# ElesionKyrie/Extreme-Video-Compression-With-Prediction-Using-Pre-trainded-Diffusion-Models-

Measured on AMD Instinct MI355X. Metric: decoded frames/sec (128x128x30) at q3, higher is better.
Workload: dtype f32

## Files before the change

### extreme-video-compression-with-prediction-using-pre-trainded-diffusion-models-_amd/build.py

```python
import os
import shutil
import subprocess
import sys
from concurrent.futures import ThreadPoolExecutor

HERE = os.path.dirname(os.path.abspath(__file__))
CSRC = os.path.join(HERE, "csrc")
LIBDIR = os.path.join(HERE, "lib")
OBJDIR = os.path.join(HERE, "build")
INCLUDE = os.path.join(os.path.dirname(HERE), "include")
HIP_SOURCES = ["conv_igemm.hip", "nin_gemm.hip", "attention.hip", "norm.hip", "fir.hip", "elementwise.hip", "gdn.hip", "stride2.hip", "lpips.hip", "i3d.hip", "frames.hip", "noise.hip", "yuv.hip", "rate.hip", "ssim.hip", "metric.hip", "inception.hip", "resample.hip", "tile.hip", "api.hip"]
ARCH = "gfx950"


def _newer(target, deps):
    if not os.path.exists(target):
        return True
    t = os.path.getmtime(target)
    return any(os.path.getmtime(d) > t for d in deps)


def _run(cmd):
    r = subprocess.run(cmd, capture_output=True, text=True)
    if r.returncode != 0:
        raise RuntimeError("build failed: %s\n%s\n%s" % (" ".join(cmd), r.stdout, r.stderr))


def hipcc_path():
    for c in (os.environ.get("HIPCC"), shutil.which("hipcc"), "/opt/rocm/bin/hipcc"):
        if c and os.path.exists(c):
            return c
    raise RuntimeError("hipcc not found (ROCm toolchain required to build libevc_hip.so)")


# ... 34 lines not shown
```

### extreme-video-compression-with-prediction-using-pre-trainded-diffusion-models-_amd/lib.py

```python
import ctypes
import math
import os
from ctypes import POINTER, c_char_p, c_double, c_float, c_int, c_int32, c_longlong, c_uint, c_uint8, c_ulonglong, c_void_p

import numpy as np
import torch

HERE = os.path.dirname(os.path.abspath(__file__))
HIP_SO = os.path.join(HERE, "lib", "libevc_hip.so")
if os.environ.get("EVC_HIP_SO"):
    HIP_SO = os.path.abspath(os.environ["EVC_HIP_SO"])
RANS_SO = os.path.join(HERE, "lib", "libevc_rans.so")

ACT_NONE, ACT_SILU, ACT_RELU = 0, 1, 2
ARITH_F32, ARITH_BF16X6, ARITH_F16X3 = 0, 1, 2
_ARITH_NAMES = {"f32": ARITH_F32, "bf16x6": ARITH_BF16X6, "f16x3": ARITH_F16X3}
_ARITH_DTYPES = {ARITH_F32: torch.float32, ARITH_BF16X6: torch.bfloat16, ARITH_F16X3: torch.float16}


def _arith_policy():
    name = os.environ.get("EVC_CONV_ARITH", "f16x3").lower()
    if name not in _ARITH_NAMES:
        raise ValueError(f"EVC_CONV_ARITH must be one of {sorted(_ARITH_NAMES)}, got {name!r}")
    return _ARITH_NAMES[name]
# ... 24 lines not shown
                ("out_scale", c_float), ("act_out", c_int),
                ("out", c_void_p), ("ld_out", c_int),
                ("B", c_int), ("H", c_int), ("W", c_int), ("Co", c_int), ("KH", c_int), ("KW", c_int),
                ("splits", c_int), ("stats_out", c_void_p), ("arith", c_int), ("in_bound", c_void_p),
                ("x2_src0", c_void_p), ("x2_src1", c_void_p), ("x2_C0", c_int), ("x2_C1", c_int), ("x2_ld0", c_int),
                ("x2_ld1", c_int), ("x2_w_packed", c_void_p), ("x2_bound", c_void_p), ("invariant", c_int)]


class ConvPlan(ctypes.Structure):
    _fields_ = [("kernel", ctypes.c_char * 96), ("tile_m", c_int), ("tile_n", c_int), ("splits", c_int),
                ("steps_per_split", c_int), ("cut_chunk", c_int), ("tail_tiles", c_int), ("tail_splits", c_int),
                ("stats_runs", c_int), ("fused_1x1", c_int)]


class NinArgs(ctypes.Structure):
    _fields_ = [("x", c_void_p), ("x1", c_void_p), ("Ci", c_int), ("Co", c_int), ("coef_a", c_void_p), ("coef_s", c_void_p),
                ("in_bound", c_void_p), ("w_packed", c_void_p), ("arith", c_int), ("bias", c_void_p), ("res", c_void_p),
                ("out_scale", c_float), ("act_out", c_int), ("out", c_void_p), ("stats_out", c_void_p),
                ("B", c_int), ("H", c_int), ("W", c_int), ("tile", c_int)]


class NinPlan(ctypes.Structure):
    _fields_ = [("kernel", ctypes.c_char * 64), ("tile_m", c_int), ("tile_n", c_int), ("stages", c_int), ("stats_runs", c_int)]


class AttentionPlan(ctypes.Structure):
    _fields_ = [("kernel", ctypes.c_char * 64), ("waves", c_int), ("kparts", c_int), ("tiles_per_part", c_int),
                ("kv_planes", c_int), ("merge", c_int), ("short_seq", c_int),
                ("lds_bytes", c_longlong), ("parts_bytes", c_longlong), ("ws_bytes", c_longlong)]


HIP_SYMBOLS = {
    "evc_version": (c_char_p, []),
    "evc_arch": (c_char_p, []),
    "evc_device_ok": (c_int, []),
    "evc_clock_probe": (c_int, [c_void_p, c_int, c_void_p, c_void_p]),
    "evc_im2col_nchw_f32": (c_int, [c_void_p, c_void_p] + [c_int] * 9 + [c_void_p, c_void_p, c_void_p]),
    "evc_maxpool3s2_nhwc_f32": (c_int, [c_void_p, c_void_p, c_int, c_int, c_int, c_int, c_void_p]),
    "evc_lpips_layer_f32": (c_int, [c_void_p, c_void_p, c_void_p, c_void_p, c_int, c_int, c_int, c_int, c_void_p]),
    "evc_maxpool2d_nhwc_f32": (c_int, [c_void_p, c_void_p] + [c_int] * 7 + [c_void_p]),
    "evc_lpips_map_f32": (c_int, [c_void_p, c_void_p, c_void_p, c_void_p, c_int, c_int, c_int, c_void_p]),
    "evc_lpips_map_mean_f32": (c_int, [c_void_p, c_void_p, c_int, c_int, c_int, c_void_p]),
    "evc_lpips_upsample_add_f32": (c_int, [c_void_p, c_void_p] + [c_int] * 6 + [c_void_p]),
    "evc_i3d_stem_im2col_f32": (c_int, [c_void_p, c_void_p] + [c_int] * 17 + [c_void_p]),
    "evc_maxpool3d_same_nthwc_f32": (c_int, [c_void_p, c_void_p] + [c_int] * 11 + [c_void_p]),
    "evc_i3d_head_f32": (c_int, [c_void_p] * 4 + [c_int] * 6 + [c_void_p]),
# ... 42 lines not shown
    "evc_gdn_workspace_bytes": (c_longlong, [c_int, c_int, c_int, c_int]),
    "evc_gdn_f32": (c_int, [c_void_p, c_void_p, c_int, c_void_p, c_void_p, c_void_p, c_int, c_int, c_int, c_int, c_int,
                            c_int, c_void_p]),
    "evc_affine_act_nhwc_f32": (c_int, [c_void_p, c_void_p, c_void_p, c_void_p, c_int, c_int, c_int, c_int, c_int,
                                        c_int, c_void_p]),
    "evc_conv_co_pad": (c_int, [c_int]),
    "evc_conv_packed_floats": (c_longlong, [c_int, c_int, c_int, c_int]),
    "evc_conv_pack_weights_f32": (c_int, [c_void_p, c_void_p, c_int, c_int, c_int, c_int, c_void_p]),
    "evc_conv_packed_bytes": (c_longlong, [c_int, c_int, c_int, c_int, c_int]),
    "evc_conv_pack_weights": (c_int, [c_void_p, c_void_p, c_int, c_int, c_int, c_int, c_int, c_void_p]),
    "evc_conv_set_option": (c_int, [c_char_p, c_int]),
    "evc_spade_act_nhwc_f32": (c_int, [c_void_p, c_void_p, c_void_p, c_void_p, c_int, c_void_p, c_void_p, c_int, c_void_p,
                                       c_void_p, c_int, c_void_p, c_int, c_int, c_int, c_int, c_int, c_void_p]),
    "evc_conv_choose_splits": (c_int, [POINTER(ConvArgs)]),
    "evc_conv_kernel_name": (c_int, [POINTER(ConvArgs), c_char_p, c_int]),
    "evc_conv_fused_1x1_supported": (c_int, [POINTER(ConvArgs)]),
    "evc_conv_stats_splits": (c_int, [POINTER(ConvArgs)]),
    "evc_conv_workspace_bytes": (c_longlong, [POINTER(ConvArgs)]),
    "evc_conv2d_nhwc_f32": (c_int, [POINTER(ConvArgs), c_void_p, c_void_p]),
    "evc_conv2d_nhwc_profiled_f32": (c_int, [POINTER(ConvArgs), c_void_p, c_void_p, c_void_p, c_void_p]),
    "evc_nin_gemm_supported": (c_int, [POINTER(NinArgs)]),
    "evc_nin_gemm_plan_query": (c_int, [POINTER(NinArgs), POINTER(NinPlan)]),
    "evc_nin_gemm_f32": (c_int, [POINTER(NinArgs), c_void_p]),
    "evc_attention_f32": (c_int, [c_void_p, c_void_p, c_void_p, c_int, c_void_p, c_int, c_int, c_int, c_int, c_int,
                                  c_float, c_void_p]),
    "evc_attention_workspace_bytes": (c_longlong, [c_int, c_int, c_int, c_int]),
    "evc_attention_set_option": (c_int, [c_char_p, c_int]),
    "evc_attention_plan_query": (c_int, [c_int, c_int, c_int, c_int, c_int, c_int, c_int, POINTER(AttentionPlan)]),
    "evc_attention_ws_f32": (c_int, [c_void_p, c_void_p, c_void_p, c_int, c_void_p, c_int, c_int, c_int, c_int, c_int,
                                     c_float, c_void_p, c_void_p]),
    "evc_frame_group_norm_f32": (c_int, [c_void_p] * 4 + [c_int] * 5 + [c_float, c_void_p]),
    "evc_frame_attention_f32": (c_int, [c_void_p, c_int, c_void_p, c_int] + [c_int] * 5 + [c_float, c_void_p]),
    "evc_frame_mix_f32": (c_int, [c_void_p] * 4 + [c_int] * 3 + [c_longlong, c_void_p]),
    "evc_frame_taps_f32": (c_int, [c_void_p, c_void_p] + [c_int] * 4 + [c_void_p]),
    "evc_ddpm_step_f32": (c_int, [c_void_p, c_void_p, c_void_p, c_longlong] + [c_float] * 5 + [c_int, c_void_p]),
    "evc_ddim_step_f32": (c_int, [c_void_p, c_void_p, c_longlong] + [c_float] * 4 + [c_int, c_void_p]),
    "evc_axpy_f32": (c_int, [c_void_p, c_void_p, c_void_p, c_longlong, c_float, c_void_p]),
    "evc_pndm_transfer_f32": (c_int, [c_void_p, c_void_p, c_void_p, c_longlong, c_float, c_float, c_float, c_int,
                                      c_void_p]),
    "evc_lincomb4_f32": (c_int, [c_void_p] * 5 + [c_longlong] + [c_float] * 4 + [c_void_p]),
    "evc_scale_clamp_f32": (c_int, [c_void_p, c_void_p, c_longlong, c_float, c_float, c_int, c_float, c_float,
                                    c_void_p]),
    "evc_gate_residual_f32": (c_int, [c_void_p, c_void_p, c_void_p, c_void_p, c_longlong, c_void_p]),
    "evc_elic_gather_params_f32": (c_int, [c_void_p] + [c_int] * 8 + [c_void_p, c_int, c_void_p, c_void_p,
                                                                       c_void_p]),
    "evc_elic_scatter_symbols_f32": (c_int, [c_void_p, c_void_p, c_void_p] + [c_int] * 7 + [c_void_p]),
# ... 717 lines not shown
    L = hip_lib()
    B, H, W, Ci = x.shape
    assert x.is_contiguous() and x.dtype == torch.float32 and (res is None or (res.is_contiguous() and res.shape == (B, H, W, Co)))
    if out is None:
        out = torch.empty((B, H, W, Co), device=x.device, dtype=torch.float32)
    assert out.is_contiguous() and out.shape == (B, H, W, Co)
    ca, cs = coef if coef is not None else (None, None)
    assert ca is None or (ca.shape == (B, Ci) and cs.shape == (B, Ci) and ca.is_contiguous() and cs.is_contiguous())
    a = NinArgs(x=ptr(x), x1=None, Ci=Ci, Co=Co, coef_a=ptr(ca), coef_s=ptr(cs), in_bound=_word(in_bound),
                w_packed=ptr(w_packed), arith=packed_arith(w_packed), bias=ptr(bias), res=ptr(res), out_scale=float(out_scale),
                act_out=ACT_NONE, out=ptr(out), B=B, H=H, W=W, tile=tile)
    plan = NinPlan()
    _check(L.evc_nin_gemm_plan_query(ctypes.byref(a), ctypes.byref(plan)), "evc_nin_gemm_plan_query")
    stats = None
    if want_stats:
        stats = torch.empty((B, plan.stats_runs, Co, 2), device=x.device, dtype=torch.float32)
        a.stats_out = ptr(stats)
    _check(L.evc_nin_gemm_f32(ctypes.byref(a), stream_ptr()), "evc_nin_gemm_f32")
    if NIN_PROFILE is not None:
        NIN_PROFILE.append(dict(kernel=plan.kernel.decode(), tile=(plan.tile_m, plan.tile_n), shape=(B, H, W, Ci, Co),
                                coef=coef is not None, bound=in_bound is not None, res=res is not None, stats=bool(want_stats)))
    return (out, stats) if want_stats else out


def attention_set_option(name, value):
    if hip_lib(require_device=False).evc_attention_set_option(name.encode(), int(value)) != 0:
        raise EvcKernelError(f"unknown attention option {name!r}")


ATTN_PROFILE = None


def attention_plan(B, heads, N, D, with_bounds=False, have_ws=None, invariant=False):
    L = hip_lib(require_device=False)
    if have_ws is None:
        nbytes = (L.evc_attention_invariant_workspace_bytes if invariant else L.evc_attention_workspace_bytes)(B, heads, N, D)
        have_ws = nbytes > 0
    out = AttentionPlan()
    _check(L.evc_attention_plan_query(B, heads, N, D, int(bool(with_bounds)), int(bool(have_ws)), int(bool(invariant)),
                                      ctypes.byref(out)), "evc_attention_plan_query")
    return dict(kernel=out.kernel.decode(), waves=out.waves, kparts=out.kparts, tiles_per_part=out.tiles_per_part,
                kv_planes=bool(out.kv_planes), merge=bool(out.merge), short_seq=bool(out.short_seq),
                lds_bytes=out.lds_bytes, parts_bytes=out.parts_bytes, ws_bytes=out.ws_bytes)


def attention(qkv, C, heads, out=None, bounds=None, invariant=False, ws=None):
# ... 537 lines not shown
```

### extreme-video-compression-with-prediction-using-pre-trainded-diffusion-models-_amd/scorenet.py

```python
import math
from types import SimpleNamespace

import numpy as np
import torch

from . import lib as L

FIR_K = np.outer([1, 3, 3, 1], [1, 3, 3, 1]).astype(np.float32)
FIR_K /= FIR_K.sum()
INV_SQRT2 = float(np.float32(1.0) / np.sqrt(np.float32(2.0)))


def num_groups(ch):
    g = min(ch // 4, 32)
    while ch % g != 0:
        g -= 1
    return g


def dims_from_config(config):
    m, d = config.model, config.data
    return SimpleNamespace(ngf=m.ngf, ch_mult=list(m.ch_mult), num_res_blocks=m.num_res_blocks,
                           attn_resolutions=list(m.attn_resolutions), n_head_channels=m.n_head_channels,
                           image_size=d.image_size, channels=d.channels, num_frames=d.num_frames,
# ... 180 lines not shown
        self._unfused = set()
        self._site_of = {}
        self._set_site_args()
        self.demote_seconds = 0.0
        self._rows = {}
        self._row_tensors = {}
        self._table = torch.zeros((256, self.ss_total), device=self.device, dtype=torch.float32)
        self._n_rows = 0
        self.use_graphs = use_graphs
        self._graphs = {}
        self._f16_raw = L.bounded_arith() == L.ARITH_F16X3
        import os
        self.overlap_skip = os.environ.get("EVC_OVERLAP_SKIP", "1") != "0"
        self.fuse_skip = self._f16_raw and os.environ.get("EVC_FUSE_SKIP", "1") != "0"
        self._side_streams = {}
        self._bounds_by_stream = {}
        self._bounds = None
        self._bound_next = 0
        self._bound_batch = 1
        if demote:
            self.demote(demote)

    def _conv(self, *a, **kw):
        return L.conv2d_nhwc(*a, invariant=self.batch_invariant, **kw)

    def _act(self, t, stats=None):
        return _Act(t, stats, invariant=self.batch_invariant)

    def _gn(self, *a, **kw):
        return L.gn_coeffs(*a, invariant=self.batch_invariant, **kw)

    def _mbound(self, *a, **kw):
        return L.moments_bound(*a, invariant=self.batch_invariant, **kw)

    def _attention(self, *a, **kw):
        return L.attention(*a, invariant=self.batch_invariant, **kw)

    def _fuse_ok(self, *a, **kw):
        return L.conv_fused_1x1_supported(*a, invariant=self.batch_invariant, **kw)

    def invariant_view(self):
        import copy
        if self.batch_invariant:
            return self
        if self.SPADE or self.ARCH != "unetmore" or self.noise_in_cond:
            raise NotImplementedError("batch_invariant is built for the concat-conditioned score network (ScoreNet) only")
        if self._demoted:
# ... 286 lines not shown
        if qkvb is None:
            obound = None
            qkv = self._proj(x.t, e["wqkv"], 3 * C, e["bqkv"], coef=coef)
        else:
            qkv, qst = self._proj(x.t, e["wqkv"], 3 * C, e["bqkv"], coef=coef, want_stats=True)
            self._mbound(qst, 0, C, qkvb, site=self._site("attn_qkv", i))
            obound = _f16_only(e["wo"], qkvb.view(B, 3)[:, 2].contiguous() if self.batch_invariant else qkvb[2:3])
        o = self._attention(qkv.view(B, H * W, 3 * C), C, heads, bounds=None if i in self._attn_f32 else qkvb)
        return self._act(*self._proj(o.view(B, H, W, C), e["wo"], C, e["bo"], res=x.t, out_scale=INV_SQRT2, want_stats=True,
                                     in_bound=obound))

    nin_gemm = True

    def _proj(self, x, w, Co, bias, coef=None, res=None, out_scale=1.0, want_stats=False, in_bound=None):
        B, H, W, Ci = x.shape
        plain = not self.batch_invariant and not self.SPADE and self.ARCH == "unetmore"
        if self.nin_gemm and plain and L.packed_arith(w) == L.ARITH_F16X3 and \
                L.nin_gemm_supported(B, H, W, Ci, Co, coef=coef is not None, bound=in_bound is not None):
            return L.nin_gemm(x, w, Co, bias=bias, coef=coef, res=res, out_scale=out_scale, in_bound=in_bound,
                              want_stats=want_stats)
        return self._conv(x, w, Co, 1, 1, bias=bias, coef=coef, res=res, out_scale=out_scale, want_stats=want_stats,
                          in_bound=in_bound)

    @torch.no_grad()
    def forward_rows(self, x, rows, cond=None):
        if self.batch_invariant and self._demoted:
            raise ValueError("batch-invariant mode does not combine with demoted sites (range recovery)")
        return self._forward_rows(x, rows, cond)

    def _forward_rows(self, x, rows, cond=None):
        d = self.d
        prog = self.program
        B, _, H, W = x.shape
        self._bound_batch = B if self.batch_invariant else 1
        nb = 256 * self._bound_batch
        if self._f16_raw:
            if torch.cuda.is_current_stream_capturing():
                self._bounds = torch.empty(nb, device=self.device, dtype=torch.int32)
            else:
                key = torch.cuda.current_stream().cuda_stream
                self._bounds = self._bounds_by_stream.get(key)
                if self._bounds is None or self._bounds.numel() != nb:
                    self._bounds = self._bounds_by_stream[key] = torch.empty(nb, device=self.device, dtype=torch.int32)
            self._bounds.zero_()
            self._bound_next = 0
        taps = getattr(self, "taps", None)
# ... 119 lines not shown
```

### include/evc_hip.h

```cpp
#ifndef EVC_HIP_H
#define EVC_HIP_H

#ifdef __cplusplus
extern "C" {
#endif

#define EVC_OK 0
#define EVC_EINVAL (-1)
#define EVC_EUNSUPPORTED (-2)
#define EVC_ELAUNCH (-3)

#define EVC_ACT_NONE 0
#define EVC_ACT_SILU 1
#define EVC_ACT_RELU 2

#define EVC_ARITH_F32 0
#define EVC_ARITH_BF16X6 1
#define EVC_ARITH_F16X3 2

const char* evc_version(void);
const char* evc_arch(void);
int evc_device_ok(void);

int evc_clock_probe(unsigned long long* out2, int spin_us, const unsigned* stop, void* stream);
// ... 93 lines not shown

int evc_conv2d_nhwc_profiled_f32(const evc_conv_args* a, float* ws, void* stream, void* ev_start, void* ev_conv_end);

typedef struct {
    const float* x; const float* x1;
    int Ci; int Co;
    const float* coef_a; const float* coef_s;
    const unsigned* in_bound;
    const float* w_packed; int arith;
    const float* bias; const float* res;
    float out_scale; int act_out;
    float* out; float* stats_out;
    int B; int H; int W;
    int tile;
} evc_nin_args;
typedef struct {
    char kernel[64];
    int tile_m, tile_n, stages, stats_runs;
} evc_nin_plan;
int evc_nin_gemm_supported(const evc_nin_args* a);
int evc_nin_gemm_plan_query(const evc_nin_args* a, evc_nin_plan* out);
int evc_nin_gemm_f32(const evc_nin_args* a, void* stream);

int evc_attention_f32(const float* q, const float* k, const float* v, int ld_qkv, float* out, int ld_out, int B,
                      int heads, int N, int D, float scale, void* stream);
long long evc_attention_workspace_bytes(int B, int heads, int N, int D);
int evc_attention_set_option(const char* name, int value);
int evc_attention_ws_f32(const float* q, const float* k, const float* v, int ld_qkv, float* out, int ld_out, int B,
                         int heads, int N, int D, float scale, float* ws, void* stream);

int evc_attention_f16x3_f32(const float* q, const float* k, const float* v, int ld_qkv, float* out, int ld_out, int B,
                            int heads, int N, int D, float scale, const unsigned* bounds, float* ws, void* stream);

typedef struct {
    char kernel[64];
    int waves, kparts, tiles_per_part, kv_planes, merge, short_seq;
    long long lds_bytes, parts_bytes, ws_bytes;
} evc_attention_plan;
int evc_attention_plan_query(int B, int heads, int N, int D, int with_bounds, int have_ws, int invariant,
                             evc_attention_plan* out);

int evc_frame_group_norm_f32(const float* x, float* y, const float* gamma, const float* beta, int B, int N, int HW, int C,
                             int groups, float eps, void* stream);
int evc_frame_attention_f32(const float* qkv, int ld_qkv, float* out, int ld_out, int B, int N, int HW, int C, int heads,
                            float scale, void* stream);
int evc_frame_mix_f32(const float* x, float* y, const float* w, const float* bias, int B, int N, int M, long long inner,
// ... 112 lines not shown
```

Before: 37.86.

## Add specialized small-spatial 3x3 conv kernel with split-K across waves

Adds a dedicated HIP kernel for 3x3 convolutions on small spatial maps that tiles 64 output pixels per workgroup, splits the channel dimension across four waves with an LDS cross-wave reduction, double-buffers activations in LDS and prefetches weights per tap. It also fuses the affine+SiLU input transform, an optional extra 1x1 (x2) input path, residual and stats into the kernel. ScoreNet now routes eligible f16x3 3x3 convs to this kernel instead of the generic implicit-GEMM path. The aim is to cut under-occupancy and launch inefficiency of the generic kernel on small, low-workgroup-count layers. The risk is extra reduction and synchronisation overhead and heuristics that pick poorly for some shapes.

Result: no change. 38.24, median of 6 (+1.0%).

```diff
diff --git a/extreme-video-compression-with-prediction-using-pre-trainded-diffusion-models-_amd/build.py b/extreme-video-compression-with-prediction-using-pre-trainded-diffusion-models-_amd/build.py
--- a/extreme-video-compression-with-prediction-using-pre-trainded-diffusion-models-_amd/build.py
+++ b/extreme-video-compression-with-prediction-using-pre-trainded-diffusion-models-_amd/build.py
@@ -9,7 +9,7 @@
 LIBDIR = os.path.join(HERE, "lib")
 OBJDIR = os.path.join(HERE, "build")
 INCLUDE = os.path.join(os.path.dirname(HERE), "include")
-HIP_SOURCES = ["conv_igemm.hip", "nin_gemm.hip", "attention.hip", "norm.hip", "fir.hip", "elementwise.hip", "gdn.hip", "stride2.hip", "lpips.hip", "i3d.hip", "frames.hip", "noise.hip", "yuv.hip", "rate.hip", "ssim.hip", "metric.hip", "inception.hip", "resample.hip", "tile.hip", "api.hip"]
+HIP_SOURCES = ["conv_igemm.hip", "nin_gemm.hip", "conv_small.hip", "attention.hip", "norm.hip", "fir.hip", "elementwise.hip", "gdn.hip", "stride2.hip", "lpips.hip", "i3d.hip", "frames.hip", "noise.hip", "yuv.hip", "rate.hip", "ssim.hip", "metric.hip", "inception.hip", "resample.hip", "tile.hip", "api.hip"]
 ARCH = "gfx950"
 
 
diff --git a/extreme-video-compression-with-prediction-using-pre-trainded-diffusion-models-_amd/csrc/conv_small.hip b/extreme-video-compression-with-prediction-using-pre-trainded-diffusion-models-_amd/csrc/conv_small.hip
--- /dev/null
+++ b/extreme-video-compression-with-prediction-using-pre-trainded-diffusion-models-_amd/csrc/conv_small.hip
@@ -0,0 +1,493 @@
+#include <hip/hip_runtime.h>
+#include <stdint.h>
+#include <stdio.h>
+#include <type_traits>
+#include "../../include/evc_hip.h"
+#include "split_mfma.h"
+
+namespace {
+
+constexpr int SMALL_PLAIN = 0, SMALL_AFFINE_SILU = 2;
+constexpr int SMALL_SR = 108;
+constexpr int SMALL_RB = 32;
+constexpr int SMALL_PLANE = SMALL_SR * SMALL_RB;
+constexpr int SMALL_STEP = 2 * SMALL_PLANE + 32;
+constexpr int SMALL_BUF = 4 * SMALL_STEP;
+constexpr int SMALL_LDS = 2 * SMALL_BUF;
+constexpr int SMALL_LDS_CAP = 80 * 1024;
+constexpr int SMALL_RED = 4 * 2 * 16 * 64 * 4;
+static_assert(SMALL_RED <= SMALL_LDS, "the cross-wave sum reuses the staging buffers");
+
+struct SmallK {
+    const float* src0; const float* src1; int C0, C1, ld0, ld1;
+    const float* coef_a; const float* coef_s;
+    const char* w; const float* w_hdr; const unsigned* in_bound;
+    const float* bias; const float* res; int ld_res; float out_scale;
+    float* out; int ld_out; float* stats;
+    const float* x2_src0; const float* x2_src1; int x2_C0, x2_C1, x2_ld0, x2_ld1;
+    const char* x2_w; const float* x2_hdr; const unsigned* x2_bound;
+    int H, W, lw, HW, Co, CoPad, nchunk, nstage, nchunk2, nstage2;
+    int npt, order;
+};
+
+__device__ __forceinline__ float small_silu(float v) { return v * __builtin_amdgcn_rcpf(1.0f + __expf(-v)); }
+
+template <int MODE>
+__device__ __forceinline__ float4 small_transform(float4 v, const float4& a, const float4& s, bool ok) {
+    if (MODE == SMALL_AFFINE_SILU) {
+        v.x = v.x * a.x + s.x; v.y = v.y * a.y + s.y; v.z = v.z * a.z + s.z; v.w = v.w * a.w + s.w;
+        v.x = small_silu(v.x); v.y = small_silu(v.y); v.z = small_silu(v.z); v.w = small_silu(v.w);
+    }
+    v.x = ok ? v.x : 0.f; v.y = ok ? v.y : 0.f; v.z = ok ? v.z : 0.f; v.w = ok ? v.w : 0.f;
+    return v;
+}
+
+__device__ __forceinline__ void small_pin(float4& v) { asm volatile("" : "+v"(v.x), "+v"(v.y), "+v"(v.z), "+v"(v.w)); }
+
+template <bool RES, bool STATS>
+__device__ __forceinline__ void small_epilogue(const SmallK& p, const f32x16& acc, float ascale, int mb, int co, int half) {
+    const float oscale = p.out_scale;
+    const float bias = p.bias ? p.bias[co] : 0.f;
+    float st_sum = 0.f, st_sq = 0.f;
+    float rv[16];
+#pragma unroll
+    for (int r = 0; r < 16; ++r) rv[r] = 0.f;
+    if (RES) {
+        const float* rp = p.res + (size_t)(mb + 4 * half) * p.ld_res + co;
+#pragma unroll
+        for (int r = 0; r < 16; ++r) rv[r] = rp[(size_t)((r & 3) + 8 * (r >> 2)) * p.ld_res];
+    }
+    float* o = p.out + (size_t)(mb + 4 * half) * p.ld_out + co;
+#pragma unroll
+    for (int r = 0; r < 16; ++r) {
+        const float v = (acc[r] * ascale + bias + rv[r]) * oscale;
+        o[(size_t)((r & 3) + 8 * (r >> 2)) * p.ld_out] = v;
+        if (STATS) { st_sum += v; st_sq += v * v; }
+    }
+    if (STATS) {
+        st_sum += __shfl_xor(st_sum, 32);
+        st_sq += __shfl_xor(st_sq, 32);
+        if (half == 0) {
+            float* sp = p.stats + ((size_t)(mb / 32) * p.Co + co) * 2;
+            sp[0] = st_sum; sp[1] = st_sq;
+        }
+    }
+}
+
+template <int TN, int MODE, bool X2>
+__global__ __launch_bounds__(256, 2) void conv_small_kernel(SmallK p) {
+    typedef Split<2> SP;
+    typedef SP::vec vec;
+    constexpr int RB = SMALL_RB, PLANE = SMALL_PLANE, STEP = SMALL_STEP, BUF = SMALL_BUF;
+    constexpr int NSET = TN == 3 ? 3 : 9;
+    constexpr int BD = TN == 1 ? 6 : TN == 2 ? 3 : 1;
+    extern __shared__ __attribute__((aligned(16))) char smem_small[];
+
+    const int tid = threadIdx.x;
+    const int lane = tid & 63;
+    const int wave = __builtin_amdgcn_readfirstlane(tid >> 6);
+    const int l31 = lane & 31, half = lane >> 5;
+    int ptile, ctile;
+    {
+        const int id = blockIdx.x;
+        if (p.order) {
+            const int T = gridDim.x, x = id & 7;
+            const int o = x * (T >> 3) + min(x, T & 7) + (id >> 3);
+            ctile = o / p.npt; ptile = o - ctile * p.npt;
+        } else {
+            ctile = id / p.npt; ptile = id - ctile * p.npt;
+        }
+    }
+    const int m0 = ptile * 64;
+    const int n0 = ctile * 32 * TN;
+    const int W = p.W, lw = p.lw, W2 = W + 2;
+    const int smp = m0 / p.HW;
+    const int y0 = (m0 - smp * p.HW) >> lw;
+    const int npx = 64 + 2 * W;
+
+    const int pc = tid & 7, sc = pc >> 1, skh = pc & 1, prow = tid >> 3;
+    const int sr0 = (prow >> lw) * W2 + (prow & (W - 1)) + 1;
+    const int srstep = (32 >> lw) * W2;
+    unsigned okm = 0;
+#pragma unroll
+    for (int j = 0; j < 3; ++j) {
+        const int pi = prow + 32 * j;
+        const int y = y0 + (pi >> lw) - 1;
+        okm |= ((pi < npx && y >= 0 && y < p.H) ? 1u : 0u) << j;
+        okm |= (unsigned)(((sr0 + j * srstep) >> 3) & 1) << (4 + j);
+    }
+    const bool wr2 = prow < 2 * W;
+    const unsigned pix0 = (unsigned)(m0 - W + prow);
+    const int a_wr0 = sc * STEP + sr0 * RB + 16 * skh;
+    const int fbase0 = (l31 >> lw) * W2 + (l31 & (W - 1));
+    const unsigned wlane = (unsigned)((n0 + l31) * RB + 16 * (half ^ ((l31 >> 3) & 1)));
+    const unsigned wq = (unsigned)p.CoPad * RB;
+
+    float4 areg[3][2];
+    const std::integral_constant<int, 0> J0; const std::integral_constant<int, 3> J3;
+    const std::integral_constant<int, (TN == 3 ? 2 : 3)> JA;
+    auto load_a = [&](int s, const float* s0, const float* s1, int C0, int ld0, int ld1, auto j0, auto j1) {
+        const int cc = s * 64;
+        const bool first = cc < C0;
+        const char* src = reinterpret_cast<const char*>(first ? s0 : s1);
+        const unsigned ld = (unsigned)(first ? ld0 : ld1);
+        const unsigned cofs = (unsigned)((first ? cc : cc - C0) + pc * 8);
+#pragma unroll
+        for (int j = decltype(j0)::value; j < decltype(j1)::value; ++j) {
+            const unsigned o = ((((okm >> j) & 1u) ? pix0 + 32u * j : (unsigned)m0) * ld + cofs) * 4u;
+            areg[j][0] = *reinterpret_cast<const float4*>(src + o);
+            areg[j][1] = *reinterpret_cast<const float4*>(src + o + 16);
+        }
+    };
+    const float* const coef_l = reinterpret_cast<const float*>(smem_small + SMALL_LDS);
+    const int Ct = p.C0 + p.C1;
+    auto store_a = [&](int buf, float xs, int s, auto mode, auto j0, auto j1) {
+        constexpr int MD = decltype(mode)::value;
+        char* A = smem_small + buf * BUF;
+        float4 ca[2], cs[2];
+        if (MD == SMALL_AFFINE_SILU) {
+            const float* c = coef_l + s * 64 + pc * 8;
+            ca[0] = *reinterpret_cast<const float4*>(c); ca[1] = *reinterpret_cast<const float4*>(c + 4);
+            cs[0] = *reinterpret_cast<const float4*>(c + Ct); cs[1] = *reinterpret_cast<const float4*>(c + Ct + 4);
+        }
+#pragma unroll
+        for (int j = decltype(j0)::value; j < decltype(j1)::value; ++j) {
+            vec pl[2];
+            small_pin(areg[j][0]); small_pin(areg[j][1]);
+            const bool ok = (okm >> j) & 1u;
+            SP::split(small_transform<MD>(areg[j][0], ca[0], cs[0], ok), small_transform<MD>(areg[j][1], ca[1], cs[1], ok), xs, pl);
+            if (j < 2 || wr2) {
+                char* d = A + a_wr0 + j * srstep * RB + (((okm >> (4 + j)) & 1u) ? (skh ? -16 : 16) : 0);
+                *reinterpret_cast<vec*>(d) = pl[0];
+                *reinterpret_cast<vec*>(d + PLANE) = pl[1];
+            }
+        }
+    };
+
+    f32x16 acc[2][TN];
+#pragma unroll
+    for (int i = 0; i < 2; ++i)
+#pragma unroll
+        for (int j = 0; j < TN; ++j)
+#pragma unroll
+            for (int r = 0; r < 16; ++r) acc[i][j][r] = 0.f;
+
+    auto kstep = [&](int buf, int toff, const vec (&bb)[TN][2]) {
+        const char* Ab = smem_small + buf * BUF + wave * STEP;
+        if constexpr (TN == 3) {
+#pragma unroll
+            for (int i = 0; i < 2; ++i) {
+                const int sr = fbase0 + i * srstep + toff;
+                const int o = sr * RB + 16 * (half ^ ((sr >> 3) & 1));
+                vec a[2];
+#pragma unroll
+                for (int q = 0; q < 2; ++q) a[q] = *reinterpret_cast<const vec*>(Ab + q * PLANE + o);
+#pragma unroll
+                for (int t = 0; t < SP::NTERM; ++t)
+#pragma unroll
+                    for (int j = 0; j < TN; ++j) acc[i][j] = SP::mfma(a[SP::qa(t)], bb[j][SP::qb(t)], acc[i][j]);
+            }
+        } else {
+            vec a[2][2];
+#pragma unroll
+            for (int i = 0; i < 2; ++i) {
+                const int sr = fbase0 + i * srstep + toff;
+                const int o = sr * RB + 16 * (half ^ ((sr >> 3) & 1));
+#pragma unroll
+                for (int q = 0; q < 2; ++q) a[i][q] = *reinterpret_cast<const vec*>(Ab + q * PLANE + o);
+            }
+#pragma unroll
+            for (int t = 0; t < SP::NTERM; ++t)
+#pragma unroll
+                for (int i = 0; i < 2; ++i)
+#pragma unroll
+                    for (int j = 0; j < TN; ++j) acc[i][j] = SP::mfma(a[i][SP::qa(t)], bb[j][SP::qb(t)], acc[i][j]);
+        }
+    };
+
+    for (int o = tid * 16; o < SMALL_LDS; o += 256 * 16) *reinterpret_cast<float4*>(smem_small + o) = make_float4(0.f, 0.f, 0.f, 0.f);
+    if (MODE == SMALL_AFFINE_SILU) {
+        float4* const cl = reinterpret_cast<float4*>(smem_small + SMALL_LDS);
+        const float4* const ga = reinterpret_cast<const float4*>(p.coef_a + (size_t)smp * Ct);
+        const float4* const gs = reinterpret_cast<const float4*>(p.coef_s + (size_t)smp * Ct);
+        for (int o = tid; o < Ct / 4; o += 256) { cl[o] = ga[o]; cl[Ct / 4 + o] = gs[o]; }
+    }
+    __syncthreads();
+
+    const float s1 = p.in_bound ? bound_scale(p.in_bound[0]) : 1.0f;
+    const float xscale = F16_ACT_SCALE * s1;
+
+    if constexpr (X2) {
+        const float s2 = bound_scale(p.x2_bound[0]);
+        const float xscale2 = F16_ACT_SCALE * s2;
+        const char* const wl2 = p.x2_w + (size_t)(wave * 2 * p.CoPad) * RB + wlane;
+        const unsigned wstage2 = 8u * wq;
+        vec bc[TN][2], bn[TN][2];
+        auto load_b2 = [&](vec (&d)[TN][2], int s) {
+            const char* src = wl2 + (size_t)s * wstage2;
+#pragma unroll
+            for (int j = 0; j < TN; ++j)
+#pragma unroll
+                for (int q = 0; q < 2; ++q) d[j][q] = *reinterpret_cast<const vec*>(src + q * wq + j * 32 * RB);
+        };
+        load_a(0, p.x2_src0, p.x2_src1, p.x2_C0, p.x2_ld0, p.x2_ld1, J0, J3);
+        load_b2(bc, 0);
+        store_a(0, xscale2, 0, std::integral_constant<int, SMALL_PLAIN>(), J0, J3);
+        __syncthreads();
+        for (int s = 0; s < p.nstage2; ++s) {
+            const int buf = s & 1;
+            const int sn = min(s + 1, p.nstage2 - 1);
+            load_a(sn, p.x2_src0, p.x2_src1, p.x2_C0, p.x2_ld0, p.x2_ld1, J0, J3);
+            load_b2(bn, sn);
+            __builtin_amdgcn_sched_barrier(0);
+            kstep(buf, W2 + 1, bc);
+            __builtin_amdgcn_sched_barrier(0);
+            store_a(buf ^ 1, xscale2, sn, std::integral_constant<int, SMALL_PLAIN>(), J0, J3);
+#pragma unroll
+            for (int j = 0; j < TN; ++j)
+#pragma unroll
+                for (int q = 0; q < 2; ++q) bc[j][q] = bn[j][q];
+            __syncthreads();
+        }
+        const float r = (p.x2_hdr[0] / s2) / (p.w_hdr[0] / s1);
+#pragma unroll
+        for (int i = 0; i < 2; ++i)
+#pragma unroll
+            for (int j = 0; j < TN; ++j)
+#pragma unroll
+                for (int e = 0; e < 16; ++e) acc[i][j][e] *= r;
+    }
+
+    {
+        const char* const wl = p.w + (size_t)(wave * 2 * p.CoPad) * RB + wlane;
+        const unsigned wtap = (unsigned)p.nchunk * 2u * wq;
+        const unsigned wstage = 8u * wq;
+        vec breg[NSET][TN][2];
+        auto load_b = [&](vec (&d)[TN][2], int s, int tap) {
+            const char* src = wl + (size_t)s * wstage + (size_t)tap * wtap;
+#pragma unroll
+            for (int j = 0; j < TN; ++j)
+#pragma unroll
+                for (int q = 0; q < 2; ++q) d[j][q] = *reinterpret_cast<const vec*>(src + q * wq + j * 32 * RB);
+        };
+        load_a(0, p.src0, p.src1, p.C0, p.ld0, p.ld1, J0, J3);
+#pragma unroll
+        for (int d = 0; d < BD; ++d) load_b(breg[d], 0, d);
+        store_a(0, xscale, 0, std::integral_constant<int, MODE>(), J0, J3);
+        __syncthreads();
+        for (int s = 0; s < p.nstage; ++s) {
+            const int buf = s & 1;
+            const int sn = min(s + 1, p.nstage - 1);
+            load_a(sn, p.src0, p.src1, p.C0, p.ld0, p.ld1, J0, JA);
+            __builtin_amdgcn_sched_barrier(0);
+#pragma unroll
+            for (int tap = 0; tap < 9; ++tap) {
+                const int tp = tap + BD;
+                if (tp < 9) load_b(breg[tp % NSET], s, tp);
+                else load_b(breg[tp % NSET], sn, tp - 9);
+                __builtin_amdgcn_sched_barrier(0);
+                kstep(buf, (tap / 3) * W2 + tap % 3, breg[tap % NSET]);
+                __builtin_amdgcn_sched_barrier(0);
+                if (tap == (TN == 3 ? 3 : 4)) {
+                    store_a(buf ^ 1, xscale, sn, std::integral_constant<int, MODE>(), J0, JA);
+                    if (TN == 3) load_a(sn, p.src0, p.src1, p.C0, p.ld0, p.ld1, JA, J3);
+                }
+                if (TN == 3 && tap == 7) store_a(buf ^ 1, xscale, sn, std::integral_constant<int, MODE>(), JA, J3);
+            }
+            __syncthreads();
+        }
+    }
+
+    const float ascale = p.w_hdr[0] / s1;
+    float4* const red = reinterpret_cast<float4*>(smem_small);
+#pragma unroll
+    for (int j = 0; j < TN; ++j) {
+        if (j > 0) __syncthreads();
+#pragma unroll
+        for (int i = 0; i < 2; ++i)
+#pragma unroll
+            for (int r4 = 0; r4 < 4; ++r4)
+                red[((wave * 2 + i) * 4 + r4) * 64 + lane] =
+                    make_float4(acc[i][j][4 * r4], acc[i][j][4 * r4 + 1], acc[i][j][4 * r4 + 2], acc[i][j][4 * r4 + 3]);
+        __syncthreads();
+#pragma unroll
+        for (int i = 0; i < 2; ++i) {
+            if (wave != ((2 * j + i) & 3)) continue;
+            f32x16 sum;
+#pragma unroll
+            for (int k = 0; k < 4; ++k)
+#pragma unroll
+                for (int r4 = 0; r4 < 4; ++r4) {
+                    const float4 v = red[((k * 2 + i) * 4 + r4) * 64 + lane];
+                    if (k == 0) { sum[4 * r4] = v.x; sum[4 * r4 + 1] = v.y; sum[4 * r4 + 2] = v.z; sum[4 * r4 + 3] = v.w; }
+                    else { sum[4 * r4] += v.x; sum[4 * r4 + 1] += v.y; sum[4 * r4 + 2] += v.z; sum[4 * r4 + 3] += v.w; }
+                }
+            const int mb = m0 + i * 32, co = n0 + j * 32 + l31;
+            if (p.res) {
+                if (p.stats) small_epilogue<true, true>(p, sum, ascale, mb, co, half);
+                else small_epilogue<true, false>(p, sum, ascale, mb, co, half);
+            } else {
+                if (p.stats) small_epilogue<false, true>(p, sum, ascale, mb, co, half);
+                else small_epilogue<false, false>(p, sum, ascale, mb, co, half);
+            }
+        }
+    }
+}
+
+
+constexpr int SMALL_XCD_ORDER = 1;
+constexpr int SMALL_MIN_WGS = 160, SMALL_MAX_STAGES_W8 = 21, SMALL_MAX_STAGES_W16 = 15, SMALL_MAX_X2_STAGES = 6;
+constexpr int SMALL_CUS = 256;
+
+struct SmallLaunch {
+    int tn, mode, runs, order;
+    bool x2;
+    dim3 grid;
+    size_t lds;
+    SmallK k;
+};
+
+bool small_pick_tile(long long M, int K, int Co, int HW, int& tn) {
+    (void)K; (void)HW;
+    long long best = -1;
+    for (int c = 3; c >= 1; --c) {
+        if (Co % (32 * c) != 0) continue;
+        const long long wgs = (M / 64) * (Co / (32 * c));
+        const long long cost = ((wgs + SMALL_CUS - 1) / SMALL_CUS) * (2 * c + 1);
+        if (best < 0 || cost < best) { best = cost; tn = c; }
+    }
+    return best >= 0;
+}
+
+inline bool ld_ok(int ld, int C) { return ld == 0 || (ld >= C && (ld & 3) == 0); }
+
+int small_resolve(const evc_conv_small_args* sa, SmallLaunch& p) {
+    if (!sa) return EVC_EINVAL;
+    const evc_conv_args* a = &sa->conv;
+    if (!a->src0 || !a->w_packed || !a->out) return EVC_EINVAL;
+    if (a->B <= 0 || a->H <= 0 || a->W <= 0 || a->Co <= 0 || a->C0 <= 0 || a->C1 < 0) return EVC_EINVAL;
+    if (a->C1 > 0 && !a->src1) return EVC_EINVAL;
+    if ((a->coef_a != nullptr) != (a->coef_s != nullptr)) return EVC_EINVAL;
+    if (!ld_ok(a->ld0, a->C0) || !ld_ok(a->ld1, a->C1)) return EVC_EINVAL;
+    if (a->ld_out < a->Co || (a->res && a->ld_res < a->Co)) return EVC_EINVAL;
+    if (sa->tn < 0 || sa->tn > 3) return EVC_EINVAL;
+    if (a->arith != EVC_ARITH_F16X3 || a->KH != 3 || a->KW != 3) return EVC_EUNSUPPORTED;
+    if (a->invariant || a->act_out != EVC_ACT_NONE || a->splits > 1) return EVC_EUNSUPPORTED;
+    if (a->W != 8 && a->W != 16) return EVC_EUNSUPPORTED;
+    const long long HW = (long long)a->H * a->W, M = HW * a->B;
+    if (HW > 256 || HW % 64 != 0) return EVC_EUNSUPPORTED;
+    if (a->C0 % 64 != 0 || a->C1 % 64 != 0 || a->Co % 32 != 0) return EVC_EUNSUPPORTED;
+    if (a->coef_a) { if (a->act_in != EVC_ACT_SILU) return EVC_EUNSUPPORTED; p.mode = SMALL_AFFINE_SILU; }
+    else { if (a->act_in != EVC_ACT_NONE) return EVC_EUNSUPPORTED; p.mode = SMALL_PLAIN; }
+    SmallK& k = p.k;
+    k.C0 = a->C0; k.C1 = a->C1;
+    k.ld0 = a->ld0 > 0 ? a->ld0 : a->C0; k.ld1 = a->ld1 > 0 ? a->ld1 : (a->C1 > 0 ? a->C1 : k.ld0);
+    k.H = a->H; k.W = a->W; k.lw = a->W == 8 ? 3 : 4; k.HW = (int)HW; k.Co = a->Co; k.CoPad = evc_conv_co_pad(a->Co);
+    k.nchunk = (a->C0 + a->C1) / 16; k.nstage = (a->C0 + a->C1) / 64;
+    k.ld_res = a->ld_res; k.ld_out = a->ld_out;
+    const long long lim = 1LL << 32;
+    if (M * k.ld0 * 4 >= lim || M * k.ld1 * 4 >= lim || M * a->ld_out * 4 >= lim || (a->res && M * a->ld_res * 4 >= lim)) return EVC_EUNSUPPORTED;
+    if (9LL * k.nchunk * 2 * k.CoPad * 32 >= lim) return EVC_EUNSUPPORTED;
+    p.x2 = a->x2_w_packed != nullptr;
+    k.x2_C0 = k.x2_C1 = k.x2_ld0 = k.x2_ld1 = k.nchunk2 = k.nstage2 = 0;
+    if (p.x2) {
+        if (!a->x2_src0 || !a->x2_bound || a->x2_C0 <= 0 || a->x2_C1 < 0 || (a->x2_C1 > 0 && !a->x2_src1)) return EVC_EINVAL;
+        if (!ld_ok(a->x2_ld0, a->x2_C0) || !ld_ok(a->x2_ld1, a->x2_C1)) return EVC_EINVAL;
+        if (a->x2_C0 % 64 != 0 || a->x2_C1 % 64 != 0) return EVC_EUNSUPPORTED;
+        k.x2_C0 = a->x2_C0; k.x2_C1 = a->x2_C1;
+        k.x2_ld0 = a->x2_ld0 > 0 ? a->x2_ld0 : a->x2_C0;
+        k.x2_ld1 = a->x2_ld1 > 0 ? a->x2_ld1 : (a->x2_C1 > 0 ? a->x2_C1 : k.x2_ld0);
+        k.nchunk2 = (a->x2_C0 + a->x2_C1) / 16; k.nstage2 = k.nchunk2 / 4;
+        if (M * k.x2_ld0 * 4 >= lim || M * k.x2_ld1 * 4 >= lim) return EVC_EUNSUPPORTED;
+    }
+    if (sa->tn) {
+        if (a->Co % (32 * sa->tn) != 0) return EVC_EUNSUPPORTED;
+        p.tn = sa->tn;
+    } else {
+        if (!small_pick_tile(M, a->C0 + a->C1, a->Co, (int)HW, p.tn)) return EVC_EUNSUPPORTED;
+        const long long wgs = (M / 64) * (a->Co / (32 * p.tn));
+        if (!sa->any_grid) {
+            if (wgs < SMALL_MIN_WGS || wgs > SMALL_CUS) return EVC_EUNSUPPORTED;
+            if (k.nstage > (a->W == 8 ? SMALL_MAX_STAGES_W8 : SMALL_MAX_STAGES_W16) || k.nstage2 > SMALL_MAX_X2_STAGES) return EVC_EUNSUPPORTED;
+        }
+    }
+    p.runs = (int)HW / 32;
+    p.lds = (size_t)SMALL_LDS + (p.mode == SMALL_AFFINE_SILU ? (size_t)(a->C0 + a->C1) * 8 : 0);
+    if (p.lds > (size_t)SMALL_LDS_CAP) return EVC_EUNSUPPORTED;
+    if (sa->order < 0 || sa->order > 2) return EVC_EINVAL;
+    p.order = sa->order ? sa->order - 1 : SMALL_XCD_ORDER;
+    k.npt = (int)(M / 64); k.order = p.order;
+    p.grid = dim3((unsigned)((M / 64) * (a->Co / (32 * p.tn))));
+    return EVC_OK;
+}
+
+int small_kernel_name(const SmallLaunch& p, char* buf, int n) {
+    return snprintf(buf, n, "conv_small_kernel<%d, %d, %s>", p.tn, p.mode, p.x2 ? "true" : "false");
+}
+
+int small_ensure_lds(const void* fn, unsigned long long* done_mask, size_t lds) {
+    if (lds <= 64 * 1024) return EVC_OK;
+    int dev = 0;
+    if (hipGetDevice(&dev) != hipSuccess) return EVC_ELAUNCH;
+    const unsigned long long bit = 1ULL << (dev & 63);
+    if (__atomic_load_n(done_mask, __ATOMIC_ACQUIRE) & bit) return EVC_OK;
+    if (hipFuncSetAttribute(fn, hipFuncAttributeMaxDynamicSharedMemorySize, SMALL_LDS_CAP) != hipSuccess) return EVC_ELAUNCH;
+    __atomic_fetch_or(done_mask, bit, __ATOMIC_RELEASE);
+    return EVC_OK;
+}
+
+template <int TN, int MODE, bool X2>
+int small_launch_one(const SmallLaunch& p, hipStream_t st) {
+    static unsigned long long done = 0;
+    const int rc = small_ensure_lds(reinterpret_cast<const void*>(&conv_small_kernel<TN, MODE, X2>), &done, p.lds);
+    if (rc != EVC_OK) return rc;
+    hipLaunchKernelGGL((conv_small_kernel<TN, MODE, X2>), p.grid, dim3(256), p.lds, st, p.k);
+    return EVC_OK;
+}
+
+template <int TN>
+int small_launch(const SmallLaunch& p, hipStream_t st) {
+    if (p.mode == SMALL_AFFINE_SILU) return p.x2 ? small_launch_one<TN, SMALL_AFFINE_SILU, true>(p, st) : small_launch_one<TN, SMALL_AFFINE_SILU, false>(p, st);
+    return p.x2 ? small_launch_one<TN, SMALL_PLAIN, true>(p, st) : small_launch_one<TN, SMALL_PLAIN, false>(p, st);
+}
+
+}
+
+extern "C" int evc_conv3x3_small_supported(const evc_conv_small_args* a) {
+    SmallLaunch p;
+    return small_resolve(a, p) == EVC_OK ? 1 : 0;
+}
+
+extern "C" int evc_conv3x3_small_plan_query(const evc_conv_small_args* a, evc_conv_small_plan* out) {
+    SmallLaunch p;
+    const int rc = !out ? EVC_EINVAL : small_resolve(a, p);
+    if (rc != EVC_OK) return rc;
+    small_kernel_name(p, out->kernel, (int)sizeof(out->kernel));
+    out->tile_m = 64; out->tile_n = 32 * p.tn; out->stages = p.k.nstage; out->x2_stages = p.k.nstage2;
+    out->workgroups = (int)p.grid.x; out->xcd_order = p.order; out->stats_runs = p.runs; out->lds_bytes = (int)p.lds;
+    return EVC_OK;
+}
+
+extern "C" int evc_conv3x3_small_f32(const evc_conv_small_args* sa, void* stream) {
+    SmallLaunch p;
+    const int rc = small_resolve(sa, p);
+    if (rc != EVC_OK) return rc;
+    const evc_conv_args* a = &sa->conv;
+    SmallK& k = p.k;
+    k.src0 = a->src0; k.src1 = a->src1 ? a->src1 : a->src0;
+    k.coef_a = a->coef_a; k.coef_s = a->coef_s; k.in_bound = a->in_bound;
+    k.w_hdr = a->w_packed;
+    k.w = reinterpret_cast<const char*>(a->w_packed) + F16_HDR_BYTES;
+    k.bias = a->bias; k.res = a->res; k.out_scale = a->out_scale; k.out = a->out; k.stats = a->stats_out;
+    k.x2_src0 = k.x2_src1 = nullptr; k.x2_w = nullptr; k.x2_hdr = nullptr; k.x2_bound = nullptr;
+    if (p.x2) {
+        k.x2_src0 = a->x2_src0; k.x2_src1 = a->x2_src1 ? a->x2_src1 : a->x2_src0;
+        k.x2_hdr = a->x2_w_packed;
+        k.x2_w = reinterpret_cast<const char*>(a->x2_w_packed) + F16_HDR_BYTES;
+        k.x2_bound = a->x2_bound;
+    }
+    hipStream_t st = (hipStream_t)stream;
+    const int lrc = p.tn == 3 ? small_launch<3>(p, st) : p.tn == 2 ? small_launch<2>(p, st) : small_launch<1>(p, st);
+    if (lrc != EVC_OK) return lrc;
+    return hipGetLastError() == hipSuccess ? EVC_OK : EVC_ELAUNCH;
+}
diff --git a/extreme-video-compression-with-prediction-using-pre-trainded-diffusion-models-_amd/lib.py b/extreme-video-compression-with-prediction-using-pre-trainded-diffusion-models-_amd/lib.py
--- a/extreme-video-compression-with-prediction-using-pre-trainded-diffusion-models-_amd/lib.py
+++ b/extreme-video-compression-with-prediction-using-pre-trainded-diffusion-models-_amd/lib.py
@@ -70,6 +70,15 @@
 
 class NinPlan(ctypes.Structure):
     _fields_ = [("kernel", ctypes.c_char * 64), ("tile_m", c_int), ("tile_n", c_int), ("stages", c_int), ("stats_runs", c_int)]
+
+
+class ConvSmallArgs(ctypes.Structure):
+    _fields_ = [("conv", ConvArgs), ("tn", c_int), ("order", c_int), ("any_grid", c_int)]
+
+
+class ConvSmallPlan(ctypes.Structure):
+    _fields_ = [("kernel", ctypes.c_char * 64), ("tile_m", c_int), ("tile_n", c_int), ("stages", c_int), ("x2_stages", c_int),
+                ("workgroups", c_int), ("stats_runs", c_int), ("lds_bytes", c_int), ("xcd_order", c_int)]
 
 
 class AttentionPlan(ctypes.Structure):
@@ -158,6 +167,9 @@
     "evc_nin_gemm_supported": (c_int, [POINTER(NinArgs)]),
     "evc_nin_gemm_plan_query": (c_int, [POINTER(NinArgs), POINTER(NinPlan)]),
     "evc_nin_gemm_f32": (c_int, [POINTER(NinArgs), c_void_p]),
+    "evc_conv3x3_small_supported": (c_int, [POINTER(ConvSmallArgs)]),
+    "evc_conv3x3_small_plan_query": (c_int, [POINTER(ConvSmallArgs), POINTER(ConvSmallPlan)]),
+    "evc_conv3x3_small_f32": (c_int, [POINTER(ConvSmallArgs), c_void_p]),
     "evc_attention_f32": (c_int, [c_void_p, c_void_p, c_void_p, c_int, c_void_p, c_int, c_int, c_int, c_int, c_int,
                                   c_float, c_void_p]),
     "evc_attention_workspace_bytes": (c_longlong, [c_int, c_int, c_int, c_int]),
@@ -921,6 +933,92 @@
                                 coef=coef is not None, bound=in_bound is not None, res=res is not None, stats=bool(want_stats)))
     return (out, stats) if want_stats else out
 
+SMALL_PROFILE = None
+
+
+def conv3x3_small_query_args(B, H, W, C0, C1, Co, arith=ARITH_F16X3, coef=True, act_in=None, bound=False, x2=(0, 0), tn=0,
+                             K=3, act_out=ACT_NONE, invariant=False, splits=0, order=0, any_grid=False):
+    act_in = (ACT_SILU if coef else ACT_NONE) if act_in is None else act_in
+    c = conv_query_args(B, H, W, C0, C1, Co, K, K, arith, coef, act_in, splits, 0, invariant)
+    c.act_out = act_out
+    d = c_void_p(16)
+    if bound:
+        c.in_bound = d
+    if x2[0] or x2[1]:
+        c.x2_src0, c.x2_C0, c.x2_w_packed, c.x2_bound = d, x2[0], d, d
+        if x2[1]:
+            c.x2_src1, c.x2_C1 = d, x2[1]
+    return ConvSmallArgs(conv=c, tn=tn, order=order, any_grid=int(bool(any_grid)))
+
+
+def conv3x3_small_supported(B, H, W, C0, C1, Co, **kw):
+    a = conv3x3_small_query_args(B, H, W, C0, C1, Co, **kw)
+    return bool(hip_lib(require_device=False).evc_conv3x3_small_supported(ctypes.byref(a)))
+
+
+def _small_plan_dict(out):
+    return dict(kernel=out.kernel.decode(), tile=(out.tile_m, out.tile_n), stages=out.stages, x2_stages=out.x2_stages,
+                workgroups=out.workgroups, stats_runs=out.stats_runs, lds_bytes=out.lds_bytes, xcd_order=bool(out.xcd_order))
+
+
+def conv3x3_small_plan(B, H, W, C0, C1, Co, **kw):
+    out = ConvSmallPlan()
+    a = conv3x3_small_query_args(B, H, W, C0, C1, Co, **kw)
+    _check(hip_lib(require_device=False).evc_conv3x3_small_plan_query(ctypes.byref(a), ctypes.byref(out)),
+           "evc_conv3x3_small_plan_query")
+    return _small_plan_dict(out)
+
+
+def conv3x3_small(src0, w_packed, Co, bias=None, src1=None, coef=None, act_in=ACT_NONE, res=None, out_scale=1.0, out=None,
+                  want_stats=False, in_bound=None, x2=None, tn=0, order=0, any_grid=False):
+    L = hip_lib()
+    p0, C0, ld0, shp = _src(src0)
+    p1, C1, ld1, shp1 = _src(src1)
+    assert shp1 is None or tuple(shp1) == tuple(shp)
+    B, H, W = shp
+    dev = (src0.t if isinstance(src0, Cols) else src0).device
+    if out is None:
+        out = torch.empty((B, H, W, Co), device=dev, dtype=torch.float32)
+    po, Cout, ldo, shpo = _src(out)
+    assert tuple(shpo) == (B, H, W) and Cout >= Co
+    ca, cs = coef if coef is not None else (None, None)
+    c = ConvArgs(p0, p1, C0, C1, ld0, ld1, ptr(ca), ptr(cs), act_in, ptr(w_packed), ptr(bias), ptr(res),
+                 0 if res is None else res.shape[-1], float(out_scale), ACT_NONE, po, ldo,
+                 B, H, W, Co, 3, 3, 0, None, packed_arith(w_packed), _word(in_bound, 1))
+    x2_ci = 0
+    if x2 is not None:
+        q0, qC0, qld0, qshp = _src(x2[0])
+        q1, qC1, qld1, _ = _src(x2[1])
+        assert tuple(qshp) == (B, H, W) and x2[2].dtype == torch.float16
+        c.x2_src0, c.x2_src1, c.x2_C0, c.x2_C1, c.x2_ld0, c.x2_ld1 = q0, q1, qC0, qC1, qld0, qld1
+        c.x2_w_packed, c.x2_bound = ptr(x2[2]), _word(x2[3], 1)
+        x2_ci = qC0 + qC1
+    a = ConvSmallArgs(conv=c, tn=tn, order=order, any_grid=int(bool(any_grid)))
+    plan = ConvSmallPlan()
+    _check(L.evc_conv3x3_small_plan_query(ctypes.byref(a), ctypes.byref(plan)), "evc_conv3x3_small_plan_query")
+    stats = None
+    if want_stats:
+        stats = torch.empty((B, plan.stats_runs, Co, 2), device=dev, dtype=torch.float32)
+        a.conv.stats_out = ptr(stats)
+    e0 = e1 = None
+    if CONV_PROFILE is not None:
+        st = torch.cuda.current_stream()
+        e0, e1 = torch.cuda.Event(enable_timing=True), torch.cuda.Event(enable_timing=True)
+        e0.record(st)
+    _check(L.evc_conv3x3_small_f32(ctypes.byref(a), stream_ptr()), "evc_conv3x3_small_f32")
+    call = dict(B=B, H=H, W=W, C0=C0, C1=C1, Co=Co, K=3, coef=coef is not None, act_in=act_in, res=res is not None,
+                out_scale=float(out_scale), bias=bias is not None, bound=in_bound is not None, arith=c.arith, ld_out=ldo,
+                stats=bool(want_stats), x2=x2_ci, invariant=False)
+    if CONV_PROFILE is not None:
+        e1.record(st)
+        CONV_PROFILE.append(dict(variant=conv_variant(Co), split=False, e0=e0, ec=e1, e1=e1, arith=c.arith,
+                                 kernel=plan.kernel.decode(), flops=2.0 * B * H * W * Co * (9 * (C0 + C1) + x2_ci),
+                                 shape=(B, H, W, C0 + C1, Co, 3), call=call))
+    if SMALL_PROFILE is not None:
+        SMALL_PROFILE.append(dict(_small_plan_dict(plan), shape=(B, H, W, C0 + C1, Co), call=call))
+    result = out.t if isinstance(out, Cols) else out
+    return (result, stats) if want_stats else result
+
 
 def attention_set_option(name, value):
     if hip_lib(require_device=False).evc_attention_set_option(name.encode(), int(value)) != 0:
diff --git a/extreme-video-compression-with-prediction-using-pre-trainded-diffusion-models-_amd/scorenet.py b/extreme-video-compression-with-prediction-using-pre-trainded-diffusion-models-_amd/scorenet.py
--- a/extreme-video-compression-with-prediction-using-pre-trainded-diffusion-models-_amd/scorenet.py
+++ b/extreme-video-compression-with-prediction-using-pre-trainded-diffusion-models-_amd/scorenet.py
@@ -226,7 +226,7 @@
             self.demote(demote)
 
     def _conv(self, *a, **kw):
-        return L.conv2d_nhwc(*a, invariant=self.batch_invariant, **kw)
+        return self._route_conv(*a, **kw)
 
     def _act(self, t, stats=None):
         return _Act(t, stats, invariant=self.batch_invariant)
@@ -559,6 +559,23 @@
         return self._conv(x, w, Co, 1, 1, bias=bias, coef=coef, res=res, out_scale=out_scale, want_stats=want_stats,
                           in_bound=in_bound)
 
+    small_conv = True
+
+    def _route_conv(self, src0, w, Co, KH, KW, **kw):
+        plain = not self.batch_invariant and not self.SPADE and self.ARCH == "unetmore"
+        if self.small_conv and plain and KH == 3 and KW == 3 and L.packed_arith(w) == L.ARITH_F16X3 and \
+                kw.get("act_out", L.ACT_NONE) == L.ACT_NONE and not kw.get("splits"):
+            _, C0, _, (B, H, W) = L._src(src0)
+            C1 = L._src(kw.get("src1"))[1]
+            x2 = kw.get("x2")
+            x2c = (L._src(x2[0])[1], L._src(x2[1])[1]) if x2 is not None else (0, 0)
+            if L.conv3x3_small_supported(B, H, W, C0, C1, Co, coef=kw.get("coef") is not None,
+                                         act_in=kw.get("act_in", L.ACT_NONE), bound=kw.get("in_bound") is not None, x2=x2c,
+                                         any_grid=self.small_conv == "any"):
+                kw.pop("act_out", None); kw.pop("splits", None)
+                return L.conv3x3_small(src0, w, Co, any_grid=self.small_conv == "any", **kw)
+        return L.conv2d_nhwc(src0, w, Co, KH, KW, invariant=self.batch_invariant, **kw)
+
     @torch.no_grad()
     def forward_rows(self, x, rows, cond=None):
         if self.batch_invariant and self._demoted:
diff --git a/include/evc_hip.h b/include/evc_hip.h
--- a/include/evc_hip.h
+++ b/include/evc_hip.h
@@ -139,6 +139,20 @@
 int evc_nin_gemm_plan_query(const evc_nin_args* a, evc_nin_plan* out);
 int evc_nin_gemm_f32(const evc_nin_args* a, void* stream);
 
+typedef struct {
+    evc_conv_args conv;
+    int tn;
+    int order;
+    int any_grid;
+} evc_conv_small_args;
+typedef struct {
+    char kernel[64];
+    int tile_m, tile_n, stages, x2_stages, workgroups, stats_runs, lds_bytes, xcd_order;
+} evc_conv_small_plan;
+int evc_conv3x3_small_supported(const evc_conv_small_args* a);
+int evc_conv3x3_small_plan_query(const evc_conv_small_args* a, evc_conv_small_plan* out);
+int evc_conv3x3_small_f32(const evc_conv_small_args* a, void* stream);
+
 int evc_attention_f32(const float* q, const float* k, const float* v, int ld_qkv, float* out, int ld_out, int B,
                       int heads, int N, int D, float scale, void* stream);
 long long evc_attention_workspace_bytes(int B, int heads, int N, int D);
```
